# ZhengdiYu/Arbitrary-Hands-3D-Reconstruction

Measured on NVIDIA H100. Metric: images/sec (512x512, HRNet-W32, two-hand MANO), higher is better.
Workload: dtype bf16

## Files before the change

### arbitrary-hands-3d-reconstruction_b200/csrc/conv_tc.cu

```cuda
#include "conv_block.cuh"
#include "conv_bottleneck.cuh"

namespace acr {

typedef CUresult (*PFN_encodeTiled)(CUtensorMap*, CUtensorMapDataType, cuuint32_t, void*, const cuuint64_t*,
                                    const cuuint64_t*, const cuuint32_t*, const cuuint32_t*, CUtensorMapInterleave,
                                    CUtensorMapSwizzle, CUtensorMapL2promotion, CUtensorMapFloatOOBfill);

static PFN_encodeTiled get_encode() {
  static PFN_encodeTiled fn = nullptr;
  if (!fn) {
    void* p = nullptr;
    cudaDriverEntryPointQueryResult q;
    if (cudaGetDriverEntryPoint("cuTensorMapEncodeTiled", &p, cudaEnableDefault, &q) == cudaSuccess &&
        q == cudaDriverEntryPointSuccess)
      fn = reinterpret_cast<PFN_encodeTiled>(p);
  }
  return fn;
}

static int num_sms() {
  static int n = 0;
  if (!n) {
    int dev = 0;
    if (cudaGetDevice(&dev) != cudaSuccess || cudaDeviceGetAttribute(&n, cudaDevAttrMultiProcessorCount, dev) != cudaSuccess || n <= 0) n = 132;
  }
  return n;
}

static int encode(CUtensorMap* m, int act_dtype, int rank, const void* ptr, const cuuint64_t* dims,
                  const cuuint64_t* strides, const cuuint32_t* box, int ck) {
  PFN_encodeTiled fn = get_encode();
  if (!fn) { set_error("conv_tc: cuTensorMapEncodeTiled unavailable (no CUDA driver?)"); return ACR_B200_ECUDA; }
  cuuint32_t es[5] = {1, 1, 1, 1, 1};
  const CUtensorMapSwizzle sw = ck == 64 ? CU_TENSOR_MAP_SWIZZLE_128B : (ck == 32 ? CU_TENSOR_MAP_SWIZZLE_64B : CU_TENSOR_MAP_SWIZZLE_32B);
  const CUtensorMapDataType dt = act_dtype == ACR_DT_BF16 ? CU_TENSOR_MAP_DATA_TYPE_BFLOAT16
                                 : (act_dtype == ACR_DT_TF32 ? CU_TENSOR_MAP_DATA_TYPE_UINT16 : CU_TENSOR_MAP_DATA_TYPE_FLOAT16);
  CUresult r = fn(m, dt, (cuuint32_t)rank, const_cast<void*>(ptr), dims, strides, box, es, CU_TENSOR_MAP_INTERLEAVE_NONE, sw,
                  CU_TENSOR_MAP_L2_PROMOTION_L2_256B, CU_TENSOR_MAP_FLOAT_OOB_FILL_NONE);
  if (r != CUDA_SUCCESS) { set_error("conv_tc: cuTensorMapEncodeTiled failed (%d)", (int)r); return ACR_B200_ECUDA; }
  return ACR_B200_OK;
}

static bool tma_out_enabled() {
  const char* e = getenv("ACR_B200_TMA_OUT");
  return e && atoi(e) != 0;
}

int conv_tc_prepare(const ConvArgs& a, int act_dtype, ConvTcPlan** out) {
  ACR_CHECK_ARG(a.out.H % TILE_Y == 0 && a.out.W % TILE_X == 0, "conv_tc: output %dx%d is not a multiple of the 16x16 super-tile", a.out.H, a.out.W);
  ACR_CHECK_ARG(a.in.pix_stride % 8 == 0 && a.cin_pad % 16 == 0 && a.cout_pad % 16 == 0 && a.cout_pad <= 2048 && a.cin_pad <= 2048,
                "conv_tc: channel alignment");
  const bool tf32 = act_dtype == ACR_DT_TF32;
  const int ew = tf32 ? 2 : 1;
  ACR_CHECK_ARG(a.in.dtype == (tf32 ? ACR_DT_F32 : act_dtype), "conv_tc: input dtype mismatch");
  ACR_CHECK_ARG(!tf32 || (a.out.dtype == ACR_DT_F32 && (!a.has_res || a.res.dtype == ACR_DT_F32) && !a.xpair && !a.s2x &&
                          !a.deconv && a.n_ext == 0),
                "conv_tc: the tf32 conv reads and writes fp32 tensors and has no x-paired, transposed or extra-term form");
  const int cin_pad = a.cin_pad * ew, in_stride = a.in.pix_stride * ew;
  ACR_CHECK_ARG(!a.deconv || (a.k == 4 && a.stride == 2 && a.cin_pad % 64 == 0 && !a.has_res && a.n_ext == 0 && !a.xpair &&
                              !a.s2x && !a.bias_per_image && !a.pow11_ch0 && a.out.H == 2 * a.in.H && a.out.W == 2 * a.in.W &&
                              a.in.H % TILE_Y == 0 && a.in.W % TILE_X == 0),
                "conv_tc: the transposed conv is k4 s2 p1 over whole 16x16 input tiles, 64-channel K chunks, no residual");
  ACR_CHECK_ARG(a.deconv || a.k == 1 || a.k == 3, "conv_tc: kernel size %d", a.k);
  ACR_CHECK_ARG(!a.xpair || (a.k == 3 && a.stride == 1 && a.cin_pad == 64 && a.cout_pad == 64 && a.in.pix_stride >= 64),
                "conv_tc: the x-paired form is a 3x3 stride-1 64->64 conv");
  ACR_CHECK_ARG(!a.s2x || (a.k == 3 && a.stride == 2 && a.cin_pad == 64 && a.in.pix_stride == 64 && a.in.C == 64 && !a.xpair &&
                           a.in.H == 2 * a.out.H && a.in.W == a.out.W),
                "conv_tc: the x-paired stride-2 form reads a dense 32-channel tensor as (H, W/2, 64)");
  ACR_CHECK_ARG(a.out.pix_stride % 2 == 0 && (!a.has_res || a.res.pix_stride % 2 == 0), "conv_tc: output / residual rows must hold channel pairs");
  const int ck = (cin_pad % 64 == 0) ? 64 : ((cin_pad % 32 == 0) ? 32 : 16);
  ConvTcPlan* pl = new ConvTcPlan();
  ConvTcParams& p = pl->p;
  pl->ck = ck; pl->act_dtype = act_dtype;
  p.patch_mode = (a.k == 3 && a.stride == 1) ? 1 : 0;
  p.patch1 = (p.patch_mode && ck == 64 && !a.xpair) ? 1 : 0;
  p.s2x = a.s2x ? 1 : 0;
  p.deconv = a.deconv ? 1 : 0;
  const cuuint32_t box_rows = p.s2x ? TILE_Y + 1 : ((p.patch_mode || p.deconv) ? TILE_Y + 2 : TILE_Y);
  const cuuint32_t box_cols = (p.patch1 || p.s2x || p.deconv) ? P1_PITCH : TILE_X;
  const cuuint64_t esz = 2;
  const cuuint64_t dim0 = (cuuint64_t)(cin_pad < in_stride ? cin_pad : in_stride);
  int rc = ACR_B200_OK;
  if (a.s2x) {
    for (int v = 0; v < 2 && !rc; ++v) {
      const char* ptr = static_cast<const char*>(a.in.ptr) + (size_t)v * a.in.W * in_stride * esz;
      cuuint64_t dims[4] = {dim0, (cuuint64_t)a.in.W, (cuuint64_t)a.in.H / 2, (cuuint64_t)a.batch};
      cuuint64_t str[3] = {(cuuint64_t)in_stride * esz, (cuuint64_t)2 * a.in.W * in_stride * esz,
                           (cuuint64_t)a.in.H * a.in.W * in_stride * esz};
      cuuint32_t box[4] = {(cuuint32_t)ck, box_cols, box_rows, 1};
      rc = encode(&p.tmA[v], act_dtype, 4, ptr, dims, str, box, ck);
    }
    for (int v = 2; v < 4 && !rc; ++v) p.tmA[v] = p.tmA[0];
  } else if (a.stride == 1 || a.deconv) {
    cuuint64_t dims[4] = {dim0, (cuuint64_t)a.in.W, (cuuint64_t)a.in.H, (cuuint64_t)a.batch};
    cuuint64_t str[3] = {(cuuint64_t)in_stride * esz, (cuuint64_t)a.in.W * in_stride * esz,
                         (cuuint64_t)a.in.H * a.in.W * in_stride * esz};
    cuuint32_t box[4] = {(cuuint32_t)ck, box_cols, box_rows, 1};
    rc = encode(&p.tmA[0], act_dtype, 4, a.in.ptr, dims, str, box, ck);
    for (int v = 1; v < 4 && !rc; ++v) p.tmA[v] = p.tmA[0];
  } else {
    for (int v = 0; v < 4 && !rc; ++v) {
      const int py = v >> 1, px = v & 1;
      const char* ptr = static_cast<const char*>(a.in.ptr) + ((size_t)py * a.in.W + px) * in_stride * esz;
      cuuint64_t dims[4] = {dim0, (cuuint64_t)a.in.W / 2, (cuuint64_t)a.in.H / 2, (cuuint64_t)a.batch};
      cuuint64_t str[3] = {(cuuint64_t)2 * in_stride * esz, (cuuint64_t)2 * a.in.W * in_stride * esz,
                           (cuuint64_t)a.in.H * a.in.W * in_stride * esz};
      cuuint32_t box[4] = {(cuuint32_t)ck, TILE_X, box_rows, 1};
      rc = encode(&p.tmA[v], act_dtype, 4, ptr, dims, str, box, ck);
    }
  }
  if (rc) { delete pl; return rc; }
  const int nsplit = (a.cout_pad + MAX_NSUB - 1) / MAX_NSUB;
  const int nsub = ((a.cout_pad + nsplit - 1) / nsplit + 15) / 16 * 16;
  p.n_ext = a.n_ext;
  for (int e = 0; e < a.n_ext; ++e) {
    ACR_CHECK_ARG((uintptr_t)a.ext[e].ptr % 4 == 0 && a.ext[e].pix_stride % 2 == 0 && a.out.dtype != ACR_DT_F32,
                  "conv_tc: extra term %d must be a 16-bit tensor with channel-pair aligned rows", e);
    p.ext[e] = a.ext[e].ptr; p.ext_shift[e] = a.ext_shift[e]; p.ext_stride[e] = a.ext[e].pix_stride;
    p.ext_W[e] = a.ext[e].W; p.ext_H[e] = a.ext[e].H;
  }
  p.tma_out = (tma_out_enabled() && !a.deconv && a.out.dtype != ACR_DT_F32 && nsub % 64 == 0 && (uintptr_t)a.out.ptr % 16 == 0 &&
               a.out.pix_stride % 8 == 0) ? 1 : 0;
  if (p.tma_out) {
    cuuint64_t dims[4] = {(cuuint64_t)a.cout_pad, (cuuint64_t)a.out.W, (cuuint64_t)a.out.H, (cuuint64_t)a.batch};
    cuuint64_t str[3] = {(cuuint64_t)a.out.pix_stride * esz, (cuuint64_t)a.out.W * a.out.pix_stride * esz,
                         (cuuint64_t)a.out.H * a.out.W * a.out.pix_stride * esz};
    cuuint32_t box[4] = {64, HALF_X, 8, 1};
    rc = encode(&p.tmOut, act_dtype, 4, a.out.ptr, dims, str, box, 64);
    if (rc) { delete pl; return rc; }
  }
  p.stage_out_bytes = p.tma_out ? 4u * 8192u : 0u;
  p.bias = a.bias; p.res = a.has_res ? a.res.ptr : nullptr; p.out = a.out.ptr;
  p.taps = a.deconv ? 4 : a.k * a.k; p.ksz = a.k; p.stride = a.stride; p.cchunks = cin_pad / ck; p.cin_pad = cin_pad;
  p.npad = a.cout_pad; p.nsplit = nsplit; p.nsub = nsub;
  pl->nt = nsub <= 64 ? 64 : 128;
  p.relu = a.relu; p.has_res = a.has_res; p.out_f32 = a.out.dtype == ACR_DT_F32;
  p.bias_per_image = a.bias_per_image; p.pow11_ch0 = a.pow11_ch0;
  p.xpair = a.xpair;
  const int grid_h = a.deconv ? a.in.H : a.out.H, grid_w = a.deconv ? a.in.W : a.out.W;
  p.tiles_x = grid_w / TILE_X; p.tiles_per_img = p.tiles_x * (grid_h / TILE_Y);
  p.total_tiles = p.tiles_per_img * a.batch;
  const int npar = a.deconv ? 4 : 1;
  p.Ho = a.out.H; p.Wo = a.out.W; p.out_stride = a.out.pix_stride;
  p.res_stride = a.has_res ? a.res.pix_stride : 0;
  p.a_stage_bytes = (uint32_t)(box_rows * box_cols) * ck * 2;
  const size_t b_total = (a.cout_pad <= 256 && !a.deconv) ?(size_t)p.taps * p.cchunks * a.cout_pad * ck * 2 : (size_t)1 << 40;
  p.bias_bytes = (uint32_t)(((size_t)a.cout_pad * 4 + 1023) & ~(size_t)1023);
  const size_t fixed = 1024  + p.bias_bytes + 512  + p.stage_out_bytes;
  const int nA = p.deconv ? p.cchunks : (p.s2x ? 2 : (p.patch1 ? p.cchunks : (p.patch_mode ? p.cchunks * 3 : p.taps * p.cchunks)));
  const size_t min_a = (size_t)((p.patch_mode && !p.patch1) ? 3 : 2) * (size_t)p.a_stage_bytes;
  p.b_resident = (b_total + min_a + fixed <= (size_t)SMEM_BUDGET) ? 1 : 0;
  p.b_block_bytes = (uint32_t)(p.b_resident ? a.cout_pad : pl->nt) * ck * 2;
  {
    const int taps = p.taps;
    cuuint64_t dims[2] = {(cuuint64_t)taps * cin_pad, (cuuint64_t)npar * a.cout_pad};
    cuuint64_t str[1] = {(cuuint64_t)taps * cin_pad * esz};
    cuuint32_t box[2] = {(cuuint32_t)ck, (cuuint32_t)(p.b_resident ? a.cout_pad : pl->nt)};
    rc = encode(&p.tmB, act_dtype, 2, a.w, dims, str, box, ck);
    if (rc) { delete pl; return rc; }
  }
  if (p.b_resident) {
    const int last_row = (nsplit - 1) * nsub + pl->nt;
    const size_t over = (size_t)(last_row > a.cout_pad ? last_row - a.cout_pad : 0) * ck * 2;
    p.b_region_bytes = (uint32_t)((b_total + over + 1023) & ~(size_t)1023);
    p.SB = 0;
  } else {
    p.SB = 4;
    while (p.SB > 2 && (size_t)p.SB * p.b_block_bytes + min_a + fixed > (size_t)SMEM_BUDGET) --p.SB;
    p.b_region_bytes = (uint32_t)(((size_t)p.SB * p.b_block_bytes + 1023) & ~(size_t)1023);
  }
  int SA = (int)(((size_t)SMEM_BUDGET - fixed - p.b_region_bytes) / p.a_stage_bytes);
  if (SA > 8) SA = 8;
  if (SA > 2 * nA && !p.patch1) SA = 2 * nA;
  if ((p.patch1 || p.s2x || p.deconv) && SA > 4) SA = 4;
  if (SA < 2) { set_error("conv_tc: shared memory plan does not fit (cout_pad %d, ck %d)", a.cout_pad, ck); delete pl; return ACR_B200_EINVAL; }
  p.SA = SA;
  p.pingpong = (p.b_resident && nA <= SA) ? 1 : 0;
  pl->smem = fixed + p.b_region_bytes + (size_t)SA * p.a_stage_bytes;
  const int nvt = p.total_tiles * nsplit * npar;
  pl->grid = nvt < num_sms() ? nvt : num_sms();
  *out = pl;
  return ACR_B200_OK;
}

int conv_tc_launch(const ConvTcPlan* pl, cudaStream_t st) {
  if (pl->act_dtype == ACR_DT_TF32) return conv_tc_launch_tf32(pl, st);
  const bool bf = pl->act_dtype == ACR_DT_BF16;
  switch (pl->ck) {
    case 64: return bf ? conv_tc_launch_64_bf16(pl, st) : conv_tc_launch_64_f16(pl, st);
    case 32: return conv_tc_launch_32(pl, st);
    default: return conv_tc_launch_16(pl, st);
  }
}

void conv_tc_free(ConvTcPlan* p) { delete p; }

int conv_block_prepare(const ConvArgs& a1, const ConvArgs& a2, int act_dtype, int store_mid, ConvBlockPlan** out) {
  auto is_3x3_64 = [&](const ConvArgs& a) {
    return a.k == 3 && a.stride == 1 && a.cin_pad == 64 && a.cout_pad == 64 && a.relu && !a.bias_per_image && !a.pow11_ch0 &&
           a.n_ext == 0 && !a.s2x && !a.deconv && a.in.dtype == act_dtype && a.out.dtype == act_dtype;
  };
  ACR_CHECK_ARG(act_dtype == ACR_DT_BF16 || act_dtype == ACR_DT_F16, "conv_block: 16-bit activations only");
  ACR_CHECK_ARG(is_3x3_64(a1) && is_3x3_64(a2) && !a1.has_res && a2.has_res && a1.xpair == a2.xpair,
                "conv_block: a BasicBlock of two 3x3 stride-1 64->64 convs (or their x-paired form), ReLU, residual on conv2");
  ACR_CHECK_ARG(a2.in.ptr == a1.out.ptr && a2.res.ptr == a1.in.ptr && a2.res.pix_stride == a1.in.pix_stride,
                "conv_block: conv2 must read conv1's output, with conv1's input as the residual");
  const int H = a1.in.H, W = a1.in.W;
  ACR_CHECK_ARG(a1.out.H == H && a1.out.W == W && a2.out.H == H && a2.out.W == W && H % TILE_Y == 0 && W % TILE_X == 0,
                "conv_block: %dx%d is not a multiple of the 16x16 super-tile", H, W);
  ACR_CHECK_ARG(a1.in.pix_stride % 8 == 0 && a1.in.pix_stride >= 64 && a2.out.pix_stride % 2 == 0 && a1.out.pix_stride % 2 == 0,
                "conv_block: row alignment");
  ConvBlockPlan* pl = new ConvBlockPlan();
  ConvBlockParams& p = pl->p;
  pl->act_dtype = act_dtype; pl->xpair = a1.xpair;
  const cuuint64_t esz = 2;
  int rc;
  {
    cuuint64_t dims[4] = {64, (cuuint64_t)W, (cuuint64_t)H, (cuuint64_t)a1.batch};
    cuuint64_t str[3] = {(cuuint64_t)a1.in.pix_stride * esz, (cuuint64_t)W * a1.in.pix_stride * esz,
                         (cuuint64_t)H * W * a1.in.pix_stride * esz};
    cuuint32_t box[4] = {64, BLK_PITCH, BLK_ROWS, 1};
    rc = encode(&p.tmA, act_dtype, 4, a1.in.ptr, dims, str, box, 64);
  }
  for (int c = 0; c < 2 && !rc; ++c) {
    cuuint64_t dims[2] = {9 * 64, 64};
    cuuint64_t str[1] = {9 * 64 * esz};
    cuuint32_t box[2] = {64, 64};
    rc = encode(c ? &p.tmB2 : &p.tmB1, act_dtype, 2, c ? a2.w : a1.w, dims, str, box, 64);
  }
  if (rc) { delete pl; return rc; }
  p.bias1 = a1.bias; p.bias2 = a2.bias;
  p.out = a2.out.ptr; p.mid = store_mid ? a1.out.ptr : nullptr;
  p.out_stride = a2.out.pix_stride; p.mid_stride = a1.out.pix_stride;
  p.H = H; p.W = W;
  p.tiles_x = W / TILE_X; p.tiles_per_img = p.tiles_x * (H / BLK_TILE_Y);
  p.total_tiles = p.tiles_per_img * a1.batch;
  pl->grid = p.total_tiles < num_sms() ? p.total_tiles : num_sms();
  *out = pl;
  return ACR_B200_OK;
}

void conv_block_free(ConvBlockPlan* p) { delete p; }

int conv_bottleneck_prepare(const ConvArgs& a1, const ConvArgs& a2, const ConvArgs& a3, int act_dtype, ConvBottleneckPlan** out) {
  auto plain = [&](const ConvArgs& a, int k, int cout_pad) {
    return a.k == k && a.stride == 1 && a.cout_pad == cout_pad && a.relu && !a.bias_per_image && !a.pow11_ch0 && a.n_ext == 0 &&
           !a.xpair && !a.s2x && !a.deconv && a.in.dtype == act_dtype && a.out.dtype == act_dtype;
  };
  ACR_CHECK_ARG(act_dtype == ACR_DT_BF16 || act_dtype == ACR_DT_F16, "conv_bottleneck: 16-bit activations only");
  ACR_CHECK_ARG(plain(a1, 1, 64) && plain(a2, 3, 64) && plain(a3, 1, 256) && !a1.has_res && !a2.has_res && a3.has_res &&
                    (a1.cin_pad == 64 || a1.cin_pad == 256) && a2.cin_pad == 64 && a3.cin_pad == 64 && a3.res.dtype == act_dtype,
                "conv_bottleneck: 1x1 (64 or 256) -> 64, 3x3 64 -> 64, 1x1 64 -> 256 + residual, stride 1, ReLU on all three");
  ACR_CHECK_ARG(a2.in.ptr == a1.out.ptr && a3.in.ptr == a2.out.ptr, "conv_bottleneck: each conv must read the previous one's output");
  const int H = a1.in.H, W = a1.in.W;
  ACR_CHECK_ARG(a1.out.H == H && a1.out.W == W && a2.out.H == H && a2.out.W == W && a3.out.H == H && a3.out.W == W &&
                    H % TILE_Y == 0 && W % TILE_X == 0,
                "conv_bottleneck: %dx%d is not a multiple of the 16x16 super-tile", H, W);
  ACR_CHECK_ARG(a1.in.pix_stride % 8 == 0 && a1.in.pix_stride >= a1.cin_pad && a3.out.pix_stride % 2 == 0 && a3.out.pix_stride >= 256 &&
                    a3.res.pix_stride % 2 == 0 && a3.res.pix_stride >= 256,
                "conv_bottleneck: row alignment");
  ConvBottleneckPlan* pl = new ConvBottleneckPlan();
  ConvBottleneckParams& p = pl->p;
  pl->act_dtype = act_dtype;
  const cuuint64_t esz = 2;
  int rc;
  {
    cuuint64_t dims[4] = {(cuuint64_t)a1.cin_pad, (cuuint64_t)W, (cuuint64_t)H, (cuuint64_t)a1.batch};
    cuuint64_t str[3] = {(cuuint64_t)a1.in.pix_stride * esz, (cuuint64_t)W * a1.in.pix_stride * esz,
                         (cuuint64_t)H * W * a1.in.pix_stride * esz};
    cuuint32_t box[4] = {64, BNK_PITCH, BNK_ROWS, 1};
    rc = encode(&p.tmA, act_dtype, 4, a1.in.ptr, dims, str, box, 64);
  }
  const ConvArgs* as[3] = {&a1, &a2, &a3};
  CUtensorMap* tms[3] = {&p.tmB1, &p.tmB2, &p.tmB3};
  for (int c = 0; c < 3 && !rc; ++c) {
    const ConvArgs& a = *as[c];
    const cuuint64_t kk = (cuuint64_t)a.k * a.k * a.cin_pad;
    cuuint64_t dims[2] = {kk, (cuuint64_t)a.cout_pad};
    cuuint64_t str[1] = {kk * esz};
    cuuint32_t box[2] = {64, (cuuint32_t)a.cout_pad};
    rc = encode(tms[c], act_dtype, 2, a.w, dims, str, box, 64);
  }
  if (rc) { delete pl; return rc; }
  p.bias1 = a1.bias; p.bias2 = a2.bias; p.bias3 = a3.bias;
  p.res = a3.res.ptr; p.out = a3.out.ptr;
  pl->cchunks = a1.cin_pad / 64;
  p.res_stride = a3.res.pix_stride; p.out_stride = a3.out.pix_stride;
  p.H = H; p.W = W;
  p.tiles_x = W / TILE_X; p.tiles_per_img = p.tiles_x * (H / BNK_TILE_Y);
  p.total_tiles = p.tiles_per_img * a1.batch;
  pl->grid = p.total_tiles < num_sms() ? p.total_tiles : num_sms();
  *out = pl;
  return ACR_B200_OK;
}

void conv_bottleneck_free(ConvBottleneckPlan* p) { delete p; }

}
```

### arbitrary-hands-3d-reconstruction_b200/csrc/conv_tc.cuh

```cuda
#pragma once
#include <cuda.h>
#include <stdlib.h>

#include "ops.cuh"
#include "wgmma.cuh"

namespace acr {

__device__ __forceinline__ uint32_t smem_u32(const void* p) { return (uint32_t)__cvta_generic_to_shared(p); }

__device__ __forceinline__ void mbar_init(uint32_t bar, uint32_t count) {
  asm volatile("mbarrier.init.shared::cta.b64 [%0], %1;" ::"r"(bar), "r"(count));
}
__device__ __forceinline__ void mbar_expect_tx(uint32_t bar, uint32_t bytes) {
  asm volatile("mbarrier.arrive.expect_tx.shared::cta.b64 _, [%0], %1;" ::"r"(bar), "r"(bytes) : "memory");
}
__device__ __forceinline__ void mbar_arrive(uint32_t bar) {
  asm volatile("mbarrier.arrive.shared::cta.b64 _, [%0];" ::"r"(bar) : "memory");
}
__device__ __forceinline__ bool elect_one_sync() {
  uint32_t pred;
  asm volatile("{\n.reg .pred p;\nelect.sync _|p, 0xffffffff;\nselp.u32 %0, 1, 0, p;\n}" : "=r"(pred));
  return pred != 0;
}
__device__ __forceinline__ void pdl_wait() { asm volatile("griddepcontrol.wait;" ::: "memory"); }
__device__ __forceinline__ void pdl_launch_dependents() { asm volatile("griddepcontrol.launch_dependents;" ::: "memory"); }
__device__ __forceinline__ void fence_barrier_init() { asm volatile("fence.mbarrier_init.release.cluster;" ::: "memory"); }

__device__ __forceinline__ void tma_load_4d(uint32_t dst, const CUtensorMap* map, uint32_t bar, int c0, int c1,
                                            int c2, int c3) {
  asm volatile(
      "cp.async.bulk.tensor.4d.shared::cluster.global.mbarrier::complete_tx::bytes [%0], [%1, {%3, %4, %5, %6}], [%2];"
      ::"r"(dst), "l"(map), "r"(bar), "r"(c0), "r"(c1), "r"(c2), "r"(c3)
      : "memory");
}
__device__ __forceinline__ void tma_load_2d(uint32_t dst, const CUtensorMap* map, uint32_t bar, int c0, int c1) {
  asm volatile(
      "cp.async.bulk.tensor.2d.shared::cluster.global.mbarrier::complete_tx::bytes [%0], [%1, {%3, %4}], [%2];"
      ::"r"(dst), "l"(map), "r"(bar), "r"(c0), "r"(c1)
      : "memory");
}
__device__ __forceinline__ void tma_prefetch_desc(const CUtensorMap* map) {
  asm volatile("prefetch.tensormap [%0];" ::"l"(map) : "memory");
}
__device__ __forceinline__ void tma_store_4d(const CUtensorMap* map, uint32_t src, int c0, int c1, int c2, int c3) {
  asm volatile("cp.async.bulk.tensor.4d.global.shared::cta.bulk_group [%0, {%2, %3, %4, %5}], [%1];"
               ::"l"(map), "r"(src), "r"(c0), "r"(c1), "r"(c2), "r"(c3) : "memory");
}
__device__ __forceinline__ void bulk_commit() { asm volatile("cp.async.bulk.commit_group;" ::: "memory"); }
__device__ __forceinline__ void bulk_wait_read0() { asm volatile("cp.async.bulk.wait_group.read 0;" ::: "memory"); }
__device__ __forceinline__ void bulk_wait_all() { asm volatile("cp.async.bulk.wait_group 0;" ::: "memory"); }
__device__ __forceinline__ void fence_proxy_async() { asm volatile("fence.proxy.async.shared::cta;" ::: "memory"); }
__device__ __forceinline__ void named_bar_sync(int id, int nthreads) { asm volatile("bar.sync %0, %1;" ::"r"(id), "r"(nthreads) : "memory"); }
__device__ __forceinline__ void named_bar_arrive_if(int id, int nthreads, uint32_t pred) {
  asm volatile("{\n.reg .pred p;\nsetp.ne.u32 p, %2, 0;\n@p bar.arrive %0, %1;\n}\n" ::"r"(id), "r"(nthreads), "r"(pred) : "memory");
}
template <int N> __device__ __forceinline__ void setmaxnreg_inc() { asm volatile("setmaxnreg.inc.sync.aligned.u32 %0;" ::"n"(N)); }
template <int N> __device__ __forceinline__ void setmaxnreg_dec() { asm volatile("setmaxnreg.dec.sync.aligned.u32 %0;" ::"n"(N)); }
__device__ __forceinline__ void sts32(uint32_t addr, uint32_t v) { asm volatile("st.shared.b32 [%0], %1;" ::"r"(addr), "r"(v) : "memory"); }
__device__ __forceinline__ uint64_t desc_lohi(uint32_t lo, uint32_t hi) { return ((uint64_t)hi << 32) | lo; }

template <typename T>
__device__ __forceinline__ void unpack2(uint32_t u, float& a, float& b) {
  const T* p = reinterpret_cast<const T*>(&u);
  a = to_f32<T>(p[0]);
  b = to_f32<T>(p[1]);
}
template <typename T>
__device__ __forceinline__ uint32_t pack2(float a, float b) {
  uint32_t u;
  T* p = reinterpret_cast<T*>(&u);
  p[0] = from_f32<T>(a);
  p[1] = from_f32<T>(b);
  return u;
}

constexpr int TILE_Y = 16, TILE_X = 16, HALF_X = 8;
constexpr int CONSUMER_WARPS = 16;
constexpr int PRODUCER_WARP = CONSUMER_WARPS;
constexpr int TC_THREADS = 32 * (CONSUMER_WARPS + 4);
constexpr int PRODUCER_REGS = 32, CONSUMER_REGS = 112;
static_assert(CONSUMER_WARPS * 32 * CONSUMER_REGS + 4 * 32 * PRODUCER_REGS <= (65536 / TC_THREADS) / 8 * 8 * TC_THREADS,
              "setmaxnreg split exceeds the launch allocation");
constexpr int TEAM_BAR = 5;
constexpr int MAX_NSUB = 128;
constexpr int SMEM_BUDGET = 224 * 1024;

struct ConvTcParams {
  CUtensorMap tmA[4];
  CUtensorMap tmB;
  const void* ext[3];
  int n_ext, ext_shift[3], ext_stride[3], ext_W[3], ext_H[3];
  CUtensorMap tmOut;
  int tma_out;
  uint32_t stage_out_bytes;
  const float* bias;
  const void* res;
  void* out;
  int taps, ksz, stride, cchunks, cin_pad, npad, relu, has_res, out_f32, bias_per_image, pow11_ch0;
  uint32_t bias_bytes;
  int nsplit, nsub;
  int xpair;
  int patch_mode, b_resident, SA, SB;
  int pingpong;
  int patch1;
  int s2x;
  int deconv;
  uint32_t a_stage_bytes, b_block_bytes, b_region_bytes;
  int tiles_x, tiles_per_img, total_tiles, Ho, Wo, out_stride, res_stride;
};

__device__ __forceinline__ int patch_kx(int i, int xpair) { return xpair ? (i == 0 ? 1 : (i == 1 ? 0 : 2)) : i; }

template <int CK>
struct SwizzleCfg {
  static constexpr uint32_t kRowBytes = CK * 2;
  static constexpr uint32_t kAtom = 8 * kRowBytes;
  static constexpr uint32_t kSBO_A = TILE_X * kRowBytes;
  static constexpr uint32_t kSwizzle = gmma_swizzle(kRowBytes);
};

constexpr int MODE_PATCH = 1, MODE_RESIDENT = 2, MODE_XPAIR = 4;
constexpr int MODE_P1 = 16;
constexpr int P1_PITCH = 24;
constexpr int MODE_S2X = 32;
constexpr int MODE_DECONV = 64;

template <int CK, typename T, int MODE, int NT>
__global__ void __launch_bounds__(TC_THREADS, 1) conv_tc_kernel(const __grid_constant__ ConvTcParams P) {
  using Cfg = SwizzleCfg<CK>;
  constexpr bool PATCH = (MODE & MODE_PATCH) != 0, RESIDENT = (MODE & MODE_RESIDENT) != 0, XPAIR = (MODE & MODE_XPAIR) != 0;
  constexpr bool P1 = (MODE & MODE_P1) != 0, S2X = (MODE & MODE_S2X) != 0, DECONV = (MODE & MODE_DECONV) != 0;
  constexpr int NPAR = DECONV ? 4 : 1;
  static_assert(!P1 || (PATCH && CK == 64 && !XPAIR), "the single-box form exists for CK = 64 patch convs (not x-paired)");
  static_assert(!S2X || (!PATCH && !P1 && !XPAIR && CK == 64), "the x-paired stride-2 form is a CK = 64 mode of its own");
  static_assert(!DECONV || (MODE == MODE_DECONV && CK == 64), "the transposed conv is a CK = 64 streamed-weight mode of its own");
  static_assert((NT == 64 || NT == 128) && (!XPAIR || NT == 64), "MMA width: 64 or 128 columns (x-paired convs: 64)");
  static_assert(!IsF32<T>::value || !(XPAIR || S2X || DECONV), "fp32 (tf32) operands: no x-paired, stride-2 x-paired or transposed form");
  extern __shared__ uint8_t smem_raw[];
  const uint32_t raw = smem_u32(smem_raw);
  const uint32_t base = (raw + 1023u) & ~1023u;
  const int SA = P.SA, SB = P.SB;
  const uint32_t b_base = base;
  const uint32_t a_base = base + P.b_region_bytes;
  const uint32_t stage_base = a_base + (uint32_t)SA * P.a_stage_bytes;
  const uint32_t bias_base = stage_base + P.stage_out_bytes;
  const uint32_t bar_base = bias_base + P.bias_bytes;
  auto fullA = [&](int s) { return bar_base + 8u * s; };
  auto emptyA = [&](int s) { return bar_base + 8u * (SA + s); };
  auto fullB = [&](int s) { return bar_base + 8u * (2 * SA + s); };
  auto emptyB = [&](int s) { return bar_base + 8u * (2 * SA + SB + s); };
  const uint32_t bres_bar = bar_base + 8u * (2 * SA + 2 * SB);
  const uint32_t dummy_bar = bres_bar + 8u;
  auto readyA = [&](int s) { return dummy_bar + 8u * (1 + s); };
  auto stageA = [&](int s) {
    if constexpr (IsF32<T>::value) return readyA(s);
    else return fullA(s);
  };
  float* s_bias = reinterpret_cast<float*>(smem_raw + (bias_base - raw));

  const int warp = threadIdx.x >> 5, lane = threadIdx.x & 31;
  const int nA = DECONV ? P.cchunks : (P.s2x ? 2 : (P.patch1 ? P.cchunks : (P.patch_mode ? P.cchunks * 3 : P.taps * P.cchunks)));
  const int nsub_taps = DECONV ? 4 : (P.patch1 ? 9 : (P.patch_mode ? 3 : 1));

  if (threadIdx.x == 0) {
    for (int s = 0; s < SA; ++s) { mbar_init(fullA(s), 1); mbar_init(emptyA(s), CONSUMER_WARPS); }
    for (int s = 0; s < SB; ++s) { mbar_init(fullB(s), 1); mbar_init(emptyB(s), CONSUMER_WARPS); }
    mbar_init(bres_bar, 1);
    mbar_init(dummy_bar, 1);
    if constexpr (IsF32<T>::value)
      for (int s = 0; s < SA; ++s) mbar_init(readyA(s), 3);
    fence_barrier_init();
    tma_prefetch_desc(&P.tmB);
    tma_prefetch_desc(&P.tmA[0]);
    if (P.tma_out) tma_prefetch_desc(&P.tmOut);
  }
  if (!P.bias_per_image)
    for (int i = threadIdx.x; i < P.npad; i += TC_THREADS) s_bias[i] = P.bias[i];
  __syncthreads();
  pdl_launch_dependents();

  if (warp >= CONSUMER_WARPS) {
    setmaxnreg_dec<PRODUCER_REGS>();
    if constexpr (IsF32<T>::value) {
      if (warp != PRODUCER_WARP) {
        const int ct = threadIdx.x - 32 * (PRODUCER_WARP + 1);
        int sa = 0;
        uint32_t pha = 0;
        for (int vt = blockIdx.x; vt < P.total_tiles * P.nsplit; vt += gridDim.x)
          for (int a = 0; a < nA; ++a) {
            mbar_wait_parity(fullA(sa), pha);
            {
              uint4* st = reinterpret_cast<uint4*>(smem_raw + (a_base - raw) + (uint32_t)sa * P.a_stage_bytes);
              for (uint32_t i = ct; i < P.a_stage_bytes / 16u; i += 96) {
                const float4 v = reinterpret_cast<const float4*>(st)[i];
                uint4 r;
                asm("cvt.rna.tf32.f32 %0, %1;" : "=r"(r.x) : "f"(v.x));
                asm("cvt.rna.tf32.f32 %0, %1;" : "=r"(r.y) : "f"(v.y));
                asm("cvt.rna.tf32.f32 %0, %1;" : "=r"(r.z) : "f"(v.z));
                asm("cvt.rna.tf32.f32 %0, %1;" : "=r"(r.w) : "f"(v.w));
                st[i] = r;
              }
              fence_proxy_async();
            }
            __syncwarp();
            if (lane == 0) mbar_arrive(readyA(sa));
            if (++sa == SA) { sa = 0; pha ^= 1u; }
          }
        return;
      }
    }
    if (warp != PRODUCER_WARP) return;
    if (P.b_resident && elect_one_sync()) {
      const int nblk = P.taps * P.cchunks;
      mbar_expect_tx(bres_bar, (uint32_t)nblk * P.b_block_bytes);
      for (int i = 0; i < nblk; ++i)
        tma_load_2d(b_base + (uint32_t)i * P.b_block_bytes, &P.tmB, bres_bar, (i / P.cchunks) * P.cin_pad + (i % P.cchunks) * CK, 0);
    }
    __syncwarp();
    pdl_wait();
    int sa = 0, sb = 0;
    uint32_t pha = 0, phb = 0;
    for (int vt = blockIdx.x; vt < P.total_tiles * P.nsplit * NPAR; vt += gridDim.x) {
      const int tile = vt / (P.nsplit * NPAR), vr = vt - tile * (P.nsplit * NPAR);
      const int par = DECONV ? vr / P.nsplit : 0;
      const int n_off = (vr - par * P.nsplit) * P.nsub;
      const int b_row = DECONV ? par * P.npad + n_off : n_off;
      const int n = tile / P.tiles_per_img, rem = tile % P.tiles_per_img;
      const int y0 = (rem / P.tiles_x) * TILE_Y, x0 = (rem % P.tiles_x) * TILE_X;
      for (int a = 0; a < nA; ++a) {
        int cc, view = 0, dy = 0, dx = 0, tap0;
        int nsub_a = nsub_taps;
        if (DECONV) {
          cc = a; dy = -1; dx = -1; tap0 = 0;
        } else if (P.s2x) {
          cc = 0; view = a; dy = a ? -1 : 0; dx = -1; tap0 = 0; nsub_a = a ? 6 : 3;
        } else if (P.patch1) {
          cc = a; dy = -1; dx = -1; tap0 = 0;
        } else if (P.patch_mode) {
          cc = a / 3; const int kx = patch_kx(a % 3, P.xpair);
          dy = -1; dx = kx - 1; tap0 = kx;
        } else {
          const int tap = a / P.cchunks; cc = a % P.cchunks; tap0 = tap;
          if (P.ksz == 3) {
            const int ky = tap / 3, kx = tap % 3;
            if (P.stride == 1) { dy = ky - 1; dx = kx - 1; }
            else {
              const int py = (ky == 1) ? 0 : 1, px = (kx == 1) ? 0 : 1;
              dy = (ky == 0) ? -1 : 0; dx = (kx == 0) ? -1 : 0;
              view = py * 2 + px;
            }
          }
        }
        mbar_wait_parity(emptyA(sa), pha ^ 1u);
        if (elect_one_sync()) {
          mbar_expect_tx(fullA(sa), P.a_stage_bytes);
          tma_load_4d(a_base + (uint32_t)sa * P.a_stage_bytes, &P.tmA[view], fullA(sa), cc * CK, x0 + dx, y0 + dy, n);
        }
        __syncwarp();
        if (++sa == SA) { sa = 0; pha ^= 1u; }
        if (!P.b_resident) {
          for (int sub = 0; sub < nsub_a; ++sub) {
            const int tap = DECONV ? sub : P.s2x ? (a == 0 ? 3 + sub : (sub < 3 ? sub : 3 + sub))
                                  : (P.patch1 ? (sub / 3) * 3 + patch_kx(sub % 3, P.xpair) : (P.patch_mode ? sub * 3 + tap0 : tap0));
            mbar_wait_parity(emptyB(sb), phb ^ 1u);
            if (elect_one_sync()) {
              mbar_expect_tx(fullB(sb), P.b_block_bytes);
              tma_load_2d(b_base + (uint32_t)sb * P.b_block_bytes, &P.tmB, fullB(sb), tap * P.cin_pad + cc * CK, b_row);
            }
            __syncwarp();
            if (++sb == SB) { sb = 0; phb ^= 1u; }
          }
        }
      }
    }
    return;
  }

  constexpr bool PINGPONG = RESIDENT;
  const bool pingpong = PINGPONG && P.pingpong != 0;
  setmaxnreg_inc<CONSUMER_REGS>();
  const int wg = warp >> 2, wq = warp & 3;
  const int h = wg & 1, rg = wg >> 1;
  if (RESIDENT) mbar_wait_parity(bres_bar, 0);
  pdl_wait();
  constexpr uint32_t pitch16 = ((P1 || S2X || DECONV) ? P1_PITCH * Cfg::kRowBytes : Cfg::kSBO_A) >> 4;
  const uint32_t hi_a = pitch16 | (Cfg::kSwizzle << 30);
  const uint32_t hi_b = (Cfg::kAtom >> 4) | (Cfg::kSwizzle << 30);
  const uint32_t lo_flags = 1u << 16;
  const uint32_t a_lo_base = (((a_base >> 4) & 0x3FFF) | lo_flags) + (uint32_t)h * (Cfg::kAtom >> 4) + (uint32_t)(rg * 8) * pitch16;
  const uint32_t b_lo_base0 = ((b_base >> 4) & 0x3FFF) | lo_flags;
  const uint32_t b_block16 = P.b_block_bytes >> 4, a_stage16 = P.a_stage_bytes >> 4;
  const int cchunks = P.cchunks, taps = P.taps, nsub = P.nsub;
  const bool tma_out = P.tma_out != 0;
  const bool plain = !tma_out && !P.has_res && !P.pow11_ch0 && P.n_ext == 0;
  const int wg_thread = threadIdx.x & 127;
  const uint32_t stage_wg = stage_base + (uint32_t)wg * 8192u;
  const uint32_t is_lane0 = lane == 0 ? 1u : 0u;
  float acc[NT / 2];
  uint32_t scale = 0;

  auto issue = [&](uint32_t a_tap, uint32_t b_lo, int kx) {
    if (XPAIR && kx != 1) {
      const int ks0 = kx == 0 ? 2 : 0;
#pragma unroll
      for (int ks = ks0; ks < ks0 + 2; ++ks)
        wgmma_m64k16<NT, T>(acc, desc_lohi(a_tap + ks * 2, hi_a), desc_lohi(b_lo + ks * 2, hi_b));
    } else {
#pragma unroll
      for (int ks = 0; ks < CK / 16; ++ks) {
        wgmma_m64k16<NT, T>(acc, desc_lohi(a_tap + ks * 2, hi_a), desc_lohi(b_lo + ks * 2, hi_b), scale);
        scale = 1;
      }
    }
  };
  uint32_t pend_a = dummy_bar, pend_b = dummy_bar;
  auto release = [&]() {
    __syncwarp();
    mbar_arrive_if(pend_b, is_lane0);
    mbar_arrive_if(pend_a, is_lane0);
    pend_a = pend_b = dummy_bar;
  };
  auto group_done = [&](uint32_t a_bar, uint32_t b_bar) {
    wgmma_commit();
    wgmma_wait<1>();
    release();
    pend_a = a_bar; pend_b = b_bar;
  };

  int sa = 0, sb = 0;
  uint32_t pha = 0, phb = 0;
  uint32_t xa_bar[3];
  const int nvt = P.total_tiles * P.nsplit * NPAR;
  if (pingpong && rg == 1) named_bar_arrive_if(TEAM_BAR, 512, 1u);
  for (int vt = blockIdx.x; vt < nvt; vt += gridDim.x) {
    if (pingpong) named_bar_sync(TEAM_BAR + rg, 512);
    scale = 0;
    const uint32_t b_lo_base = b_lo_base0 + (RESIDENT ? (uint32_t)((vt % P.nsplit) * nsub) * (Cfg::kRowBytes >> 4) : 0u);
    if (DECONV) {
      const int par = (vt / P.nsplit) & 3;
      const uint32_t a_par = a_lo_base + (uint32_t)(par >> 1) * pitch16 + (uint32_t)(par & 1) * (Cfg::kRowBytes >> 4);
      for (int cc = 0; cc < cchunks; ++cc) {
        mbar_wait_parity(stageA(sa), pha);
        const uint32_t a_lo = a_par + (uint32_t)sa * a_stage16;
#pragma unroll
        for (int t = 0; t < 4; ++t) {
          mbar_wait_parity(fullB(sb), phb);
          wgmma_fence();
          issue(a_lo + (uint32_t)(t >> 1) * pitch16 + (uint32_t)(t & 1) * (Cfg::kRowBytes >> 4), b_lo_base + (uint32_t)sb * b_block16, 1);
          group_done(t == 3 ? emptyA(sa) : dummy_bar, emptyB(sb));
          if (++sb == SB) { sb = 0; phb ^= 1u; }
        }
        if (++sa == SA) { sa = 0; pha ^= 1u; }
      }
    } else if (S2X) {
#pragma unroll
      for (int v = 0; v < 2; ++v) {
        mbar_wait_parity(stageA(sa), pha);
        const uint32_t a_lo = a_lo_base + (uint32_t)sa * a_stage16;
        if (RESIDENT) wgmma_fence();
#pragma unroll
        for (int t9 = 0; t9 < 6; ++t9) {
          if (v == 0 && t9 >= 3) continue;
          const int ky = v == 0 ? 1 : (t9 < 3 ? 0 : 2), kx = t9 % 3;
          const bool last = t9 == (v == 0 ? 2 : 5);
          uint32_t b_lo;
          if (RESIDENT) b_lo = b_lo_base + (uint32_t)(ky * 3 + kx) * b_block16;
          else { mbar_wait_parity(fullB(sb), phb); wgmma_fence(); b_lo = b_lo_base + (uint32_t)sb * b_block16; }
          const uint32_t a_tap = a_lo + (uint32_t)(ky == 2 ? pitch16 : 0u) + (uint32_t)(kx != 0 ? 1 : 0) * (Cfg::kRowBytes >> 4);
          const int ks0 = kx == 1 ? 0 : 2;
#pragma unroll
          for (int ks = ks0; ks < ks0 + 2; ++ks) {
            wgmma_m64k16<NT, T>(acc, desc_lohi(a_tap + ks * 2, hi_a), desc_lohi(b_lo + ks * 2, hi_b), scale);
            scale = 1;
          }
          if (!RESIDENT || last) group_done(last ? emptyA(sa) : dummy_bar, RESIDENT ? dummy_bar : emptyB(sb));
          if (!RESIDENT && ++sb == SB) { sb = 0; phb ^= 1u; }
        }
        if (++sa == SA) { sa = 0; pha ^= 1u; }
      }
    } else if (P1) {
      for (int cc = 0; cc < cchunks; ++cc) {
        mbar_wait_parity(stageA(sa), pha);
        const uint32_t a_lo = a_lo_base + (uint32_t)sa * a_stage16;
        if (RESIDENT) wgmma_fence();
#pragma unroll
        for (int ky = 0; ky < 3; ++ky) {
#pragma unroll
          for (int i = 0; i < 3; ++i) {
            const int kx = XPAIR ? (i == 0 ? 1 : (i == 1 ? 0 : 2)) : i;
            const bool last = ky == 2 && i == 2;
            const bool close = !RESIDENT || last;
            uint32_t b_lo;
            if (RESIDENT) b_lo = b_lo_base + (uint32_t)((ky * 3 + kx) * cchunks + cc) * b_block16;
            else { mbar_wait_parity(fullB(sb), phb); wgmma_fence(); b_lo = b_lo_base + (uint32_t)sb * b_block16; }
            issue(a_lo + (uint32_t)ky * pitch16 + (uint32_t)kx * (Cfg::kRowBytes >> 4), b_lo, kx);
            if (close) group_done(last ? emptyA(sa) : dummy_bar, RESIDENT ? dummy_bar : emptyB(sb));
            if (!RESIDENT && ++sb == SB) { sb = 0; phb ^= 1u; }
          }
        }
        if (++sa == SA) { sa = 0; pha ^= 1u; }
      }
    } else if (PATCH && XPAIR) {
      uint32_t a_lo[3];
#pragma unroll
      for (int i = 0; i < 3; ++i) {
        mbar_wait_parity(stageA(sa), pha);
        a_lo[i] = a_lo_base + (uint32_t)sa * a_stage16;
        xa_bar[i] = emptyA(sa);
        if (++sa == SA) { sa = 0; pha ^= 1u; }
      }
      wgmma_fence();
#pragma unroll
      for (int ky = 0; ky < 3; ++ky)
#pragma unroll
        for (int i = 0; i < 3; ++i) {
          const int kx = i == 0 ? 1 : (i == 1 ? 0 : 2);
          issue(a_lo[i] + (uint32_t)ky * pitch16, b_lo_base + (uint32_t)(ky * 3 + kx) * b_block16, kx);
        }
      wgmma_commit();
    } else if (PATCH) {
      for (int cc = 0; cc < cchunks; ++cc) {
#pragma unroll
        for (int i = 0; i < 3; ++i) {
          const int kx = XPAIR ? (i == 0 ? 1 : (i == 1 ? 0 : 2)) : i;
          mbar_wait_parity(stageA(sa), pha);
          const uint32_t a_lo = a_lo_base + (uint32_t)sa * a_stage16;
          if (RESIDENT) wgmma_fence();
#pragma unroll
          for (int sub = 0; sub < 3; ++sub) {
            uint32_t b_lo;
            if (RESIDENT) b_lo = b_lo_base + (uint32_t)((sub * 3 + kx) * cchunks + cc) * b_block16;
            else { mbar_wait_parity(fullB(sb), phb); wgmma_fence(); b_lo = b_lo_base + (uint32_t)sb * b_block16; }
            issue(a_lo + (uint32_t)sub * pitch16, b_lo, kx);
            if (!RESIDENT || sub == 2) group_done(sub == 2 ? emptyA(sa) : dummy_bar, RESIDENT ? dummy_bar : emptyB(sb));
            if (!RESIDENT && ++sb == SB) { sb = 0; phb ^= 1u; }
          }
          if (++sa == SA) { sa = 0; pha ^= 1u; }
        }
      }
    } else {
      uint32_t b_res = b_lo_base;
      for (int tap = 0; tap < taps; ++tap) {
        for (int cc = 0; cc < cchunks; ++cc) {
          mbar_wait_parity(stageA(sa), pha);
          uint32_t b_lo;
          if (RESIDENT) { b_lo = b_res; b_res += b_block16; }
          else { mbar_wait_parity(fullB(sb), phb); b_lo = b_lo_base + (uint32_t)sb * b_block16; }
          wgmma_fence();
          issue(a_lo_base + (uint32_t)sa * a_stage16, b_lo, 1);
          group_done(emptyA(sa), RESIDENT ? dummy_bar : emptyB(sb));
          if (!RESIDENT && ++sb == SB) { sb = 0; phb ^= 1u; }
          if (++sa == SA) { sa = 0; pha ^= 1u; }
        }
      }
    }
    if (PINGPONG) named_bar_arrive_if(TEAM_BAR + (rg ^ 1), 512, (pingpong && (rg == 0 || vt + (int)gridDim.x < nvt)) ? 1u : 0u);
    wgmma_wait<0>();
    release();
    if (XPAIR) {
#pragma unroll
      for (int i = 0; i < 3; ++i) mbar_arrive_if(xa_bar[i], is_lane0);
    }
    wgmma_acc_fence<NT / 2>(acc);

    const int tile = vt / (P.nsplit * NPAR), vr = vt - tile * (P.nsplit * NPAR);
    const int par = DECONV ? vr / P.nsplit : 0;
    const int n_off = (vr - par * P.nsplit) * nsub;
    const int n = tile / P.tiles_per_img, rem = tile % P.tiles_per_img;
    const int oy0 = (rem / P.tiles_x) * TILE_Y + rg * 8 + 2 * wq, ox = (rem % P.tiles_x) * TILE_X + h * HALF_X + (lane >> 2);
    const int cq = 2 * (lane & 3);
    const int ty0 = (rem / P.tiles_x) * TILE_Y + rg * 8, tx0 = (rem % P.tiles_x) * TILE_X + h * HALF_X;
    if constexpr (!IsF32<T>::value) {
      if (plain) {
        const int cols = min(nsub, P.npad - n_off);
        const float* pbias = P.bias_per_image ? P.bias + (size_t)n * P.npad + n_off : s_bias + n_off;
#pragma unroll
        for (int g = 0; g < NT / 64; ++g) {
          if (64 * g >= cols) break;
#pragma unroll
          for (int r2 = 0; r2 < 2; ++r2) {
            const int oy = oy0 + r2;
            const size_t pix = DECONV ? ((size_t)n * P.Ho + 2 * oy + (par >> 1)) * P.Wo + 2 * ox + (par & 1)
                                      : ((size_t)n * P.Ho + oy) * P.Wo + ox;
            const size_t o = pix * P.out_stride + n_off + cq;
#pragma unroll
            for (int jj = 0; jj < 8; ++jj) {
              const int j = 8 * g + jj;
              if (8 * j >= cols) break;
              const float2 b = *reinterpret_cast<const float2*>(pbias + 8 * j + cq);
              float f0 = acc[4 * j + 2 * r2] + b.x, f1 = acc[4 * j + 2 * r2 + 1] + b.y;
              if (P.relu) { f0 = fmaxf(f0, 0.f); f1 = fmaxf(f1, 0.f); }
              if (P.out_f32) *reinterpret_cast<float2*>(reinterpret_cast<float*>(P.out) + o + 8 * j) = make_float2(f0, f1);
              else *reinterpret_cast<uint32_t*>(reinterpret_cast<T*>(P.out) + o + 8 * j) = pack2<T>(f0, f1);
            }
          }
        }
        continue;
      }
    }
    const float* bsrc = P.bias_per_image ? P.bias + (size_t)n * P.npad + n_off : s_bias + n_off;
#pragma unroll
    for (int g = 0; g < NT / 64; ++g) {
      if (64 * g >= nsub) break;
      if (tma_out) {
        if (wg_thread == 0) bulk_wait_read0();
        named_bar_sync(1 + wg, 128);
      }
#pragma unroll
      for (int r2 = 0; r2 < 2; ++r2) {
        const int oy = oy0 + r2;
        const size_t pix = DECONV ? ((size_t)n * P.Ho + 2 * oy + (par >> 1)) * P.Wo + 2 * ox + (par & 1)
                                  : ((size_t)n * P.Ho + oy) * P.Wo + ox;
        const T* resp = P.has_res ? reinterpret_cast<const T*>(P.res) + pix * P.res_stride + n_off : nullptr;
        const uint32_t srow = stage_wg + (uint32_t)(16 * wq + (lane >> 2) + 8 * r2) * 128u;
#pragma unroll
        for (int jj = 0; jj < 8; ++jj) {
          const int j = 8 * g + jj;
          const int c = 8 * j + cq;
          const bool valid = 8 * j < nsub && n_off + c < P.npad;
          if (!valid && !tma_out) continue;
          float f0 = 0.f, f1 = 0.f;
          if (valid) {
            f0 = acc[4 * j + 2 * r2] + bsrc[c]; f1 = acc[4 * j + 2 * r2 + 1] + bsrc[c + 1];
            if (P.pow11_ch0 && n_off + c == 0) f0 = powf(1.1f, f0);
            if (resp) {
              float x0, x1;
              if constexpr (IsF32<T>::value) {
                const float2 r = *reinterpret_cast<const float2*>(resp + c);
                x0 = r.x; x1 = r.y;
              } else {
                unpack2<T>(*reinterpret_cast<const uint32_t*>(resp + c), x0, x1);
              }
              f0 += x0; f1 += x1;
            }
            if constexpr (!IsF32<T>::value)
            for (int e = 0; e < P.n_ext; ++e) {
              const T* xp = reinterpret_cast<const T*>(P.ext[e]) +
                            (((size_t)n * P.ext_H[e] + (oy >> P.ext_shift[e])) * P.ext_W[e] + (ox >> P.ext_shift[e])) * P.ext_stride[e] + n_off + c;
              float x0, x1;
              unpack2<T>(*reinterpret_cast<const uint32_t*>(xp), x0, x1);
              f0 += x0; f1 += x1;
            }
            if (P.relu) { f0 = fmaxf(f0, 0.f); f1 = fmaxf(f1, 0.f); }
          }
          if constexpr (IsF32<T>::value) {
            *reinterpret_cast<float2*>(reinterpret_cast<float*>(P.out) + pix * P.out_stride + n_off + c) = make_float2(f0, f1);
          } else if (tma_out) {
            sts32(srow + (((uint32_t)jj ^ (uint32_t)(lane >> 2)) << 4) + (uint32_t)cq * 2u, pack2<T>(f0, f1));
          } else if (P.out_f32) {
            *reinterpret_cast<float2*>(reinterpret_cast<float*>(P.out) + pix * P.out_stride + n_off + c) = make_float2(f0, f1);
          } else {
            *reinterpret_cast<uint32_t*>(reinterpret_cast<T*>(P.out) + pix * P.out_stride + n_off + c) = pack2<T>(f0, f1);
          }
        }
      }
      if (tma_out) {
        fence_proxy_async();
        named_bar_sync(1 + wg, 128);
        if (wg_thread == 0) {
          tma_store_4d(&P.tmOut, stage_wg, n_off + 64 * g, tx0, ty0, n);
          bulk_commit();
        }
      }
    }
  }
  if (tma_out && wg_thread == 0) bulk_wait_all();
}

struct ConvTcPlan {
  ConvTcParams p;
  int ck, act_dtype, grid, nt;
  size_t smem;
};

template <typename Kernel, typename Params>
static int launch_pdl(Kernel kernel, const Params& p, int grid, size_t smem, cudaStream_t st) {
  cudaLaunchConfig_t cfg = {};
  cfg.gridDim = dim3(grid); cfg.blockDim = dim3(TC_THREADS); cfg.dynamicSmemBytes = smem; cfg.stream = st;
  cudaLaunchAttribute attr[1];
  attr[0].id = cudaLaunchAttributeProgrammaticStreamSerialization;
  attr[0].val.programmaticStreamSerializationAllowed = 1;
  cfg.attrs = attr; cfg.numAttrs = 1;
  ACR_CHECK_CUDA(cudaLaunchKernelEx(&cfg, kernel, p));
  return ACR_B200_OK;
}

template <int CK, typename T, int MODE, int NT>
static int launch_nt(const ConvTcPlan* pl, cudaStream_t st) {
  static unsigned long long configured = 0;
  ACR_CHECK_CUDA(ensure_dynamic_smem(conv_tc_kernel<CK, T, MODE, NT>, SMEM_BUDGET, &configured));
  return launch_pdl(conv_tc_kernel<CK, T, MODE, NT>, pl->p, pl->grid, pl->smem, st);
}

template <int CK, typename T, int MODE>
static int launch_inst(const ConvTcPlan* pl, cudaStream_t st) {
  if constexpr ((MODE & MODE_XPAIR) != 0) return launch_nt<CK, T, MODE, 64>(pl, st);
  else return pl->nt == 64 ? launch_nt<CK, T, MODE, 64>(pl, st) : launch_nt<CK, T, MODE, 128>(pl, st);
}

template <int CK, typename T>
static int launch_mode(const ConvTcPlan* pl, cudaStream_t st) {
  const int mode = (pl->p.patch_mode ? MODE_PATCH : 0) | (pl->p.b_resident ? MODE_RESIDENT : 0);
  if constexpr (IsF32<T>::value) {
    if (pl->p.deconv || pl->p.s2x || pl->p.xpair) { set_error("conv_tc: no tf32 form of the transposed or x-paired convs"); return ACR_B200_EINVAL; }
    if constexpr (CK == 64)
      if (pl->p.patch1)
        return pl->p.b_resident ? launch_inst<64, T, MODE_PATCH | MODE_RESIDENT | MODE_P1>(pl, st)
                                : launch_inst<64, T, MODE_PATCH | MODE_P1>(pl, st);
  } else if constexpr (CK == 64) {
    if (pl->p.deconv) return launch_inst<64, T, MODE_DECONV>(pl, st);
    if (pl->p.s2x)
      return pl->p.b_resident ? launch_inst<64, T, MODE_RESIDENT | MODE_S2X>(pl, st) : launch_inst<64, T, MODE_S2X>(pl, st);
    if (pl->p.patch1)
      return pl->p.b_resident ? launch_inst<64, T, MODE_PATCH | MODE_RESIDENT | MODE_P1>(pl, st)
                              : launch_inst<64, T, MODE_PATCH | MODE_P1>(pl, st);
    if (pl->p.xpair) {
      if (mode != (MODE_PATCH | MODE_RESIDENT)) { set_error("conv_tc: x-paired conv needs resident weights"); return ACR_B200_EINVAL; }
      return launch_inst<64, T, MODE_PATCH | MODE_RESIDENT | MODE_XPAIR>(pl, st);
    }
  }
  if constexpr (CK == 64) {
    if (pl->p.patch_mode) { set_error("conv_tc: no three-box form of a 64-channel-chunk conv"); return ACR_B200_EINVAL; }
    return pl->p.b_resident ? launch_inst<64, T, MODE_RESIDENT>(pl, st) : launch_inst<64, T, 0>(pl, st);
  } else {
    switch (mode) {
      case 0: return launch_inst<CK, T, 0>(pl, st);
      case 1: return launch_inst<CK, T, 1>(pl, st);
      case 2: return launch_inst<CK, T, 2>(pl, st);
      default: return launch_inst<CK, T, 3>(pl, st);
    }
  }
}

int conv_tc_launch_64_bf16(const ConvTcPlan* pl, cudaStream_t st);
int conv_tc_launch_64_f16(const ConvTcPlan* pl, cudaStream_t st);
int conv_tc_launch_32(const ConvTcPlan* pl, cudaStream_t st);
int conv_tc_launch_16(const ConvTcPlan* pl, cudaStream_t st);
int conv_tc_launch_tf32(const ConvTcPlan* pl, cudaStream_t st);

}
```

Before: 2702.

## Add narrow MMA widths for small-channel 3x3 convs and vectorize epilogue stores

Narrow 16-bit patch-mode convs with fewer than 64 output channels now get kernel instances whose MMA width is 16, 32 or 48 columns instead of padding up to 64, so no tensor-core work is spent on padded columns. The direct-store epilogue also regroups four packed column pairs across each lane quad with shuffles and writes them as one 16-byte store when alignment allows. This adds more template instances and shuffle overhead, and the nsub values must be multiples of 16 or the launch returns an error.

```diff
diff --git a/arbitrary-hands-3d-reconstruction_b200/csrc/conv_tc.cu b/arbitrary-hands-3d-reconstruction_b200/csrc/conv_tc.cu
--- a/arbitrary-hands-3d-reconstruction_b200/csrc/conv_tc.cu
+++ b/arbitrary-hands-3d-reconstruction_b200/csrc/conv_tc.cu
@@ -134,8 +134,10 @@
   p.bias = a.bias; p.res = a.has_res ? a.res.ptr : nullptr; p.out = a.out.ptr;
   p.taps = a.deconv ? 4 : a.k * a.k; p.ksz = a.k; p.stride = a.stride; p.cchunks = cin_pad / ck; p.cin_pad = cin_pad;
   p.npad = a.cout_pad; p.nsplit = nsplit; p.nsub = nsub;
-  pl->nt = nsub <= 64 ? 64 : 128;
+  const bool narrow = p.patch_mode && !a.xpair && !tf32 && nsub < 64;
+  pl->nt = narrow ? nsub : (nsub <= 64 ? 64 : 128);
   p.relu = a.relu; p.has_res = a.has_res; p.out_f32 = a.out.dtype == ACR_DT_F32;
+  p.out_vec = (!p.out_f32 && (uintptr_t)a.out.ptr % 16 == 0 && a.out.pix_stride % 8 == 0) ? 1 : 0;
   p.bias_per_image = a.bias_per_image; p.pow11_ch0 = a.pow11_ch0;
   p.xpair = a.xpair;
   const int grid_h = a.deconv ? a.in.H : a.out.H, grid_w = a.deconv ? a.in.W : a.out.W;
diff --git a/arbitrary-hands-3d-reconstruction_b200/csrc/conv_tc.cuh b/arbitrary-hands-3d-reconstruction_b200/csrc/conv_tc.cuh
--- a/arbitrary-hands-3d-reconstruction_b200/csrc/conv_tc.cuh
+++ b/arbitrary-hands-3d-reconstruction_b200/csrc/conv_tc.cuh
@@ -73,6 +73,17 @@
   p[0] = from_f32<T>(a);
   p[1] = from_f32<T>(b);
   return u;
+}
+
+__device__ __forceinline__ void quad_transpose4(uint32_t* v, int lane) {
+  const bool e = (lane & 1) != 0;
+  uint32_t s0 = e ? v[0] : v[1], s1 = e ? v[2] : v[3];
+  uint32_t r0 = __shfl_xor_sync(0xffffffffu, s0, 1), r1 = __shfl_xor_sync(0xffffffffu, s1, 1);
+  if (e) { v[0] = r0; v[2] = r1; } else { v[1] = r0; v[3] = r1; }
+  const bool h = (lane & 2) != 0;
+  s0 = h ? v[0] : v[2]; s1 = h ? v[1] : v[3];
+  r0 = __shfl_xor_sync(0xffffffffu, s0, 2); r1 = __shfl_xor_sync(0xffffffffu, s1, 2);
+  if (h) { v[0] = r0; v[1] = r1; } else { v[2] = r0; v[3] = r1; }
 }
 
 constexpr int TILE_Y = 16, TILE_X = 16, HALF_X = 8;
@@ -108,6 +119,7 @@
   int deconv;
   uint32_t a_stage_bytes, b_block_bytes, b_region_bytes;
   int tiles_x, tiles_per_img, total_tiles, Ho, Wo, out_stride, res_stride;
+  int out_vec;
 };
 
 __device__ __forceinline__ int patch_kx(int i, int xpair) { return xpair ? (i == 0 ? 1 : (i == 1 ? 0 : 2)) : i; }
@@ -135,7 +147,9 @@
   static_assert(!P1 || (PATCH && CK == 64 && !XPAIR), "the single-box form exists for CK = 64 patch convs (not x-paired)");
   static_assert(!S2X || (!PATCH && !P1 && !XPAIR && CK == 64), "the x-paired stride-2 form is a CK = 64 mode of its own");
   static_assert(!DECONV || (MODE == MODE_DECONV && CK == 64), "the transposed conv is a CK = 64 streamed-weight mode of its own");
-  static_assert((NT == 64 || NT == 128) && (!XPAIR || NT == 64), "MMA width: 64 or 128 columns (x-paired convs: 64)");
+  static_assert((NT == 64 || NT == 128 || (NT % 16 == 0 && NT < 64 && PATCH && !XPAIR && !IsF32<T>::value)) &&
+                (!XPAIR || NT == 64), "MMA width: 64 or 128 columns (x-paired convs: 64), or a narrow 16-bit 3x3 layer's");
+  constexpr int NG = (NT + 63) / 64;
   static_assert(!IsF32<T>::value || !(XPAIR || S2X || DECONV), "fp32 (tf32) operands: no x-paired, stride-2 x-paired or transposed form");
   extern __shared__ uint8_t smem_raw[];
   const uint32_t raw = smem_u32(smem_raw);
@@ -476,7 +490,7 @@
         const int cols = min(nsub, P.npad - n_off);
         const float* pbias = P.bias_per_image ? P.bias + (size_t)n * P.npad + n_off : s_bias + n_off;
 #pragma unroll
-        for (int g = 0; g < NT / 64; ++g) {
+        for (int g = 0; g < NG; ++g) {
           if (64 * g >= cols) break;
 #pragma unroll
           for (int r2 = 0; r2 < 2; ++r2) {
@@ -484,15 +498,32 @@
             const size_t pix = DECONV ? ((size_t)n * P.Ho + 2 * oy + (par >> 1)) * P.Wo + 2 * ox + (par & 1)
                                       : ((size_t)n * P.Ho + oy) * P.Wo + ox;
             const size_t o = pix * P.out_stride + n_off + cq;
-#pragma unroll
-            for (int jj = 0; jj < 8; ++jj) {
-              const int j = 8 * g + jj;
-              if (8 * j >= cols) break;
+            auto pair = [&](int j) {
               const float2 b = *reinterpret_cast<const float2*>(pbias + 8 * j + cq);
               float f0 = acc[4 * j + 2 * r2] + b.x, f1 = acc[4 * j + 2 * r2 + 1] + b.y;
               if (P.relu) { f0 = fmaxf(f0, 0.f); f1 = fmaxf(f1, 0.f); }
-              if (P.out_f32) *reinterpret_cast<float2*>(reinterpret_cast<float*>(P.out) + o + 8 * j) = make_float2(f0, f1);
-              else *reinterpret_cast<uint32_t*>(reinterpret_cast<T*>(P.out) + o + 8 * j) = pack2<T>(f0, f1);
+              return make_float2(f0, f1);
+            };
+#pragma unroll
+            for (int jq = 0; jq < 8; jq += 4) {
+              const int j0 = 8 * g + jq;
+              if (j0 >= NT / 8 || 8 * j0 >= cols) break;
+              if (j0 + 3 < NT / 8 && P.out_vec && 8 * j0 + 32 <= cols) {
+                uint32_t v[4];
+#pragma unroll
+                for (int i = 0; i < 4; ++i) { const float2 f = pair(j0 + i); v[i] = pack2<T>(f.x, f.y); }
+                quad_transpose4(v, lane);
+                *reinterpret_cast<uint4*>(reinterpret_cast<T*>(P.out) + pix * P.out_stride + n_off + 8 * (j0 + (lane & 3))) =
+                    make_uint4(v[0], v[1], v[2], v[3]);
+                continue;
+              }
+#pragma unroll
+              for (int j = j0; j < j0 + 4; ++j) {
+                if (j >= NT / 8 || 8 * j >= cols) break;
+                const float2 f = pair(j);
+                if (P.out_f32) *reinterpret_cast<float2*>(reinterpret_cast<float*>(P.out) + o + 8 * j) = f;
+                else *reinterpret_cast<uint32_t*>(reinterpret_cast<T*>(P.out) + o + 8 * j) = pack2<T>(f.x, f.y);
+              }
             }
           }
         }
@@ -501,7 +532,7 @@
     }
     const float* bsrc = P.bias_per_image ? P.bias + (size_t)n * P.npad + n_off : s_bias + n_off;
 #pragma unroll
-    for (int g = 0; g < NT / 64; ++g) {
+    for (int g = 0; g < NG; ++g) {
       if (64 * g >= nsub) break;
       if (tma_out) {
         if (wg_thread == 0) bulk_wait_read0();
@@ -517,6 +548,7 @@
 #pragma unroll
         for (int jj = 0; jj < 8; ++jj) {
           const int j = 8 * g + jj;
+          if (j >= NT / 8) break;
           const int c = 8 * j + cq;
           const bool valid = 8 * j < nsub && n_off + c < P.npad;
           if (!valid && !tma_out) continue;
@@ -595,8 +627,17 @@
 
 template <int CK, typename T, int MODE>
 static int launch_inst(const ConvTcPlan* pl, cudaStream_t st) {
-  if constexpr ((MODE & MODE_XPAIR) != 0) return launch_nt<CK, T, MODE, 64>(pl, st);
-  else return pl->nt == 64 ? launch_nt<CK, T, MODE, 64>(pl, st) : launch_nt<CK, T, MODE, 128>(pl, st);
+  if constexpr ((MODE & MODE_XPAIR) != 0) {
+    return launch_nt<CK, T, MODE, 64>(pl, st);
+  } else {
+    if constexpr ((MODE & MODE_PATCH) != 0 && !IsF32<T>::value) {
+      if (pl->nt == 16) return launch_nt<CK, T, MODE, 16>(pl, st);
+      if (pl->nt == 32) return launch_nt<CK, T, MODE, 32>(pl, st);
+      if (pl->nt == 48) return launch_nt<CK, T, MODE, 48>(pl, st);
+    }
+    if (pl->nt != 64 && pl->nt != 128) { set_error("conv_tc: no instance of MMA width %d for this form", pl->nt); return ACR_B200_EINVAL; }
+    return pl->nt == 64 ? launch_nt<CK, T, MODE, 64>(pl, st) : launch_nt<CK, T, MODE, 128>(pl, st);
+  }
 }
 
 template <int CK, typename T>
```

Result: faster. 2886, median of 6 (+6.8%).
